# aelmiger/LINE-MOD-Pipeline

Hardware: AMD Instinct MI355X
Metric: detections/sec (higher is better)
Workload: dtype u8

## Files before the change

### line-mod-pipeline_amd/csrc/lm_dev_color.h

```cpp
#pragma once
#include "lm_dev.h"

namespace {

__global__ __launch_bounds__(256) void k_pyrdown(const u8* __restrict__ src0, int sw, int sh, u8* __restrict__ dst0,
                                                  int dw, int dh, size_t slot_stride) {
    const u8* src = slot_ptr(src0, slot_stride);
    u8* dst = slot_ptr(dst0, slot_stride);
    int x = blockIdx.x * 64 + (threadIdx.x & 63);
    int y = blockIdx.y * 4 + (threadIdx.x >> 6);
    if (x >= dw || y >= dh) return;
    const int K[5] = {1, 4, 6, 4, 1};
    int xs[5];
#pragma unroll
    for (int i = 0; i < 5; ++i) xs[i] = refl101(2 * x + i - 2, sw) * 3;
    int s0 = 0, s1 = 0, s2 = 0;
#pragma unroll
    for (int j = 0; j < 5; ++j) {
        const u8* row = src + (size_t)refl101(2 * y + j - 2, sh) * sw * 3;
        int r0 = 0, r1 = 0, r2 = 0;
#pragma unroll
        for (int i = 0; i < 5; ++i) {
            const u8* p = row + xs[i];
            r0 += K[i] * p[0]; r1 += K[i] * p[1]; r2 += K[i] * p[2];
// ... 536 lines not shown
            for (int e = 0; e < 4; ++e) {
                const int j = 4 * q + e, k = 16 * hh + j;
                const int d0 = k - 16 - n, d1 = k + 16 - n;
                const int w0 = (d0 % 3 == 0) ? mx_w(d0 / 3 + 3) : 0, w1 = (d1 % 3 == 0) ? mx_w(d1 / 3 + 3) : 0;
                const int m = (j & 3) + 8 * (j >> 2) + 4 * hh;
                const int yy = m >> 2, cc = m & 3;
                const int wp = cc == cco ? mx_w(yy - yo - 1) : 0, wc = cc == cco ? mx_w(yy - yo + 7) : 0;
                b0 |= (u32)w0 << (8 * e); b1 |= (u32)w1 << (8 * e); vp |= (u32)wp << (8 * e); vc |= (u32)wc << (8 * e);
            }
            T.v[lane][q] = b0; T.v[lane][4 + q] = b1; T.v[lane][8 + q] = vp; T.v[lane][12 + q] = vc;
        }
    }
    return T;
}
__device__ const MxTab g_mx_tab = mx_make_tab();
#define MX_WAVE_BYTES 128
__device__ __forceinline__ void permlane32_swap_lo(u32& a, u32& b) {
    const auto r = __builtin_amdgcn_permlane32_swap(a, b, false, false);
    a = r[0]; b = r[1];
}
__device__ __forceinline__ void d_cblur_mx_st(const u32 slot, const u32 tile, const u8* __restrict__ bgr0, int w, int h, u8* __restrict__ s0, size_t in_stride,
                                              size_t tmp_stride, int gx, int strip_rows) {
    const u8* bgr = slot_ptr_s(bgr0, in_stride, slot);
    u8* S = slot_ptr_s(s0, tmp_stride, slot);
    const int lane = (int)(threadIdx.x & 63u), wave = (int)(threadIdx.x >> 6);
    const int r = lane & 31, hh = lane >> 5;
    const int yy = r >> 2, cc = r & 3;
    const int cx = (int)(tile % (u32)gx), sy = (int)(tile / (u32)gx);
    const int W3 = w * 3;
    const int c0 = (cx * 4 + wave) * MX_WAVE_BYTES;
    if (c0 >= W3) return;
    const int Y0 = sy * strip_rows, Y1 = min(Y0 + strip_rows, h);
    const u32 pitch = (u32)W3;
    i32x4 B0, B1, BP, BC;
    {
        const u32x4* tp = reinterpret_cast<const u32x4*>(g_mx_tab.v[lane]);
        const u32x4 t0 = tp[0], t1 = tp[1], t2 = tp[2], t3 = tp[3];
        B0 = i32x4{(int)t0[0], (int)t0[1], (int)t0[2], (int)t0[3]}; B1 = i32x4{(int)t1[0], (int)t1[1], (int)t1[2], (int)t1[3]};
        BP = i32x4{(int)t2[0], (int)t2[1], (int)t2[2], (int)t2[3]}; BC = i32x4{(int)t3[0], (int)t3[1], (int)t3[2], (int)t3[3]};
    }
    const int cch = c0 + 32 * cc;
    const bool active = cch < W3;
    const bool rep_l = active && cch == 0 && hh == 0;
    const bool rep_r = active && cch + 32 == W3 && hh == 1;
    const bool edge_wave = __any(rep_l || rep_r);
    const u32 off0 = (u32)(!active ? 0 : rep_l ? 0 : cch - 16 + 16 * hh);
    const u32 off1 = (u32)(!active ? 0 : rep_r ? W3 - 16 : cch + 16 + 16 * hh);
    auto load_tile = [&](int yt, u32x4 (&A)[2]) {
        const u32 row = (u32)clampi(yt + yy, 0, h - 1) * pitch;
        u32x4 v0 = ld16(bgr + (row + off0)), v1 = ld16(bgr + (row + off1));
        if (edge_wave) {
            const u32 dl = v0[0], dr = v1[3];
            const u32 l0 = __builtin_amdgcn_perm(dl, dl, 0x02010002u), l1 = __builtin_amdgcn_perm(dl, dl, 0x00020100u), l2 = __builtin_amdgcn_perm(dl, dl, 0x01000201u);
            const u32 r0 = __builtin_amdgcn_perm(dr, dr, 0x01030201u), r1 = __builtin_amdgcn_perm(dr, dr, 0x02010302u), r2 = __builtin_amdgcn_perm(dr, dr, 0x03020103u);
            v0 = rep_l ? u32x4{l0, l1, l2, l0} : v0;
            v1 = rep_r ? u32x4{r0, r1, r2, r0} : v1;
        }
        A[0] = u32x4{v0[0] ^ 0x80808080u, v0[1] ^ 0x80808080u, v0[2] ^ 0x80808080u, v0[3] ^ 0x80808080u};
        A[1] = u32x4{v1[0] ^ 0x80808080u, v1[1] ^ 0x80808080u, v1[2] ^ 0x80808080u, v1[3] ^ 0x80808080u};
    };
    auto horizontal = [&](const u32x4 (&A)[2], i32x4& Hi, i32x4& Lo) {
        i32x16 c = {0, 0, 0, 0, 0, 0, 0, 0, 0, 0, 0, 0, 0, 0, 0, 0};
        c = __builtin_amdgcn_mfma_i32_32x32x32_i8(i32x4{(int)A[0][0], (int)A[0][1], (int)A[0][2], (int)A[0][3]}, B0, c, 0, 0, 0);
        c = __builtin_amdgcn_mfma_i32_32x32x32_i8(i32x4{(int)A[1][0], (int)A[1][1], (int)A[1][2], (int)A[1][3]}, B1, c, 0, 0, 0);
#pragma unroll
        for (int g = 0; g < 4; ++g) {
            const u32 r0 = (u32)c[4 * g], r1 = (u32)c[4 * g + 1], r2 = (u32)c[4 * g + 2], r3 = (u32)c[4 * g + 3];
            const u32 a01 = __builtin_amdgcn_perm(r1, r0, 0x05010400u), a23 = __builtin_amdgcn_perm(r3, r2, 0x05010400u);
            Lo[g] = (int)(__builtin_amdgcn_perm(a23, a01, 0x05040100u) ^ 0x80808080u);
            Hi[g] = (int)__builtin_amdgcn_perm(a23, a01, 0x07060302u);
        }
    };
    u32x4 A[2], An[2];
    i32x4 hiP, loP, hiC, loC;
    load_tile(Y0 - 4, A);
    horizontal(A, hiP, loP);
    const int steps = (Y1 - Y0 + 7) / 8;
    const int KC = 32768 + 128 * 256 + 32768 * 256;
    load_tile(Y0 + 4, A);
    const u32 so = (u32)(cch + 16 * hh);
    for (int m = 0; m < steps; ++m) {
        if (m + 1 < steps) load_tile(Y0 + 8 * (m + 1) + 4, An);
        horizontal(A, hiC, loC);
        i32x16 zh = {0, 0, 0, 0, 0, 0, 0, 0, 0, 0, 0, 0, 0, 0, 0, 0};
        i32x16 zl = {KC, KC, KC, KC, KC, KC, KC, KC, KC, KC, KC, KC, KC, KC, KC, KC};
        zh = __builtin_amdgcn_mfma_i32_32x32x32_i8(hiP, BP, zh, 0, 0, 0);
        zh = __builtin_amdgcn_mfma_i32_32x32x32_i8(hiC, BC, zh, 0, 0, 0);
        zl = __builtin_amdgcn_mfma_i32_32x32x32_i8(loP, BP, zl, 0, 0, 0);
        zl = __builtin_amdgcn_mfma_i32_32x32x32_i8(loC, BC, zl, 0, 0, 0);
        u32 D[4];
#pragma unroll
        for (int g = 0; g < 4; ++g) {
            u32 v[4];
#pragma unroll
            for (int e = 0; e < 4; ++e) v[e] = ((u32)zh[4 * g + e] << 8) + (u32)zl[4 * g + e];
            const u32 a01 = __builtin_amdgcn_perm(v[1], v[0], 0x0c0c0602u), a23 = __builtin_amdgcn_perm(v[3], v[2], 0x0c0c0602u);
            D[g] = __builtin_amdgcn_perm(a23, a01, 0x05040100u);
        }
        permlane32_swap_lo(D[0], D[2]);
        permlane32_swap_lo(D[1], D[3]);
        const int yout = Y0 + 8 * m + yy;
        if (active && yout < Y1) st16(S + ((u32)yout * pitch + so), u32x4{D[0], D[2], D[1], D[3]});
        hiP = hiC; loP = loC;
        A[0] = An[0]; A[1] = An[1];
    }
}

__global__ __launch_bounds__(256, 2) void k_cblur_mx(const u8* __restrict__ bgr0, int w, int h, u8* __restrict__ s0, size_t in_stride,
                                                     size_t tmp_stride, int gx, int gy, int strip_rows, int nslots) {
    u32 slot, tile;
    xcd_slot_tile_b(blockIdx.x, (u32)(gx * gy), (u32)nslots, slot, tile);
    d_cblur_mx_st(slot, tile, bgr0, w, h, s0, in_stride, tmp_stride, gx, strip_rows);
}
__global__ __launch_bounds__(256, 2) void k_blur_mx_pyr(const u8* __restrict__ bgr0, int w, int h, u8* __restrict__ s0, u8* __restrict__ bgr1,
                                                        size_t slot_stride, int gx, int gy, int strip_rows, int g_pyr, int nslots) {
    u32 slot, tile;
    const u32 g_blur = (u32)(gx * gy), G = g_blur + (u32)g_pyr;
    xcd_slot_tile_b(blockIdx.x, G, (u32)nslots, slot, tile);
    const u32 p1 = (tile + 1u) * (u32)g_pyr / G, p0 = tile * (u32)g_pyr / G;
    if (p1 != p0) d_pyrdown16_st<PD_STRIP>(slot, p0, bgr0, w, h, bgr1, w >> 1, h >> 1, slot_stride);
    else d_cblur_mx_st(slot, tile - p0, bgr0, w, h, s0, slot_stride, slot_stride, gx, strip_rows);
}

template <int SB>
__global__ __launch_bounds__(256, 2) void k_blur_pyr(const u8* __restrict__ bgr0, int w, int h, u8* __restrict__ s0, u8* __restrict__ bgr1,
                                                     size_t slot_stride, int g_blur, int g_pyr, int nslots, int interleave) {
    u32 slot, tile;
    xcd_slot_tile_b(blockIdx.x, (u32)(g_blur + g_pyr), (u32)nslots, slot, tile);
    if (!interleave) {
        if (tile < (u32)g_blur) d_cblur_sh_st<SB>(slot, tile, bgr0, w, h, s0, slot_stride, slot_stride);
        else d_pyrdown16_st<PD_STRIP>(slot, tile - (u32)g_blur, bgr0, w, h, bgr1, w >> 1, h >> 1, slot_stride);
        return;
    }
    const u32 G = (u32)(g_blur + g_pyr);
    const u32 p1 = (tile + 1u) * (u32)g_pyr / G, p0 = tile * (u32)g_pyr / G;
    if (p1 != p0) d_pyrdown16_st<PD_STRIP>(slot, p0, bgr0, w, h, bgr1, w >> 1, h >> 1, slot_stride);
    else d_cblur_sh_st<SB>(slot, tile - p0, bgr0, w, h, s0, slot_stride, slot_stride);
}

__device__ __forceinline__ void d_corient(const u32 vblock, const u8* __restrict__ s0, int w, int h, float thr2,
                                                  u8* __restrict__ qn0, float* __restrict__ mag0, size_t tmp_stride,
                                                  size_t mag_stride, int gblocks, int nslots) {
    u32 slot, tile;
    xcd_slot_tile_b(vblock, (u32)gblocks, (u32)nslots, slot, tile);
    const u8* S = slot_ptr_s(s0, tmp_stride, slot);
    u8* qn = slot_ptr_s(qn0, tmp_stride, slot);
    float* mag = mag0 ? slot_ptr_s(mag0, mag_stride, slot) : nullptr;
    const int ng = w >> 4;
    const int gid = (int)(tile * 256u) + (int)threadIdx.x;
    const int y = gid / ng, g = gid - y * ng;
    if (y >= h) return;
    const size_t pitch = (size_t)w * 3;
    u32 R[3][14];
#pragma unroll
    for (int j = 0; j < 3; ++j) {
        const u8* row = S + (size_t)clampi(y - 1 + j, 0, h - 1) * pitch + 48 * g;
        const u32x4 a = ld16(row), b = ld16(row + 16), c = ld16(row + 32);
        R[j][0] = g > 0 ? *reinterpret_cast<const u32*>(row - 4) : 0u;
        R[j][1] = a[0]; R[j][2] = a[1]; R[j][3] = a[2]; R[j][4] = a[3];
        R[j][5] = b[0]; R[j][6] = b[1]; R[j][7] = b[2]; R[j][8] = b[3];
        R[j][9] = c[0]; R[j][10] = c[1]; R[j][11] = c[2]; R[j][12] = c[3];
        R[j][13] = g + 1 < ng ? *reinterpret_cast<const u32*>(row + 48) : 0u;
    }
    u32 vse[14], vso[14], vde[14], vdo[14];
#pragma unroll
    for (int d = 0; d < 14; ++d) {
        const u32 e0 = R[0][d] & 0x00FF00FFu, o0 = (R[0][d] >> 8) & 0x00FF00FFu;
        const u32 e1 = R[1][d] & 0x00FF00FFu, o1 = (R[1][d] >> 8) & 0x00FF00FFu;
        const u32 e2 = R[2][d] & 0x00FF00FFu, o2 = (R[2][d] >> 8) & 0x00FF00FFu;
        vse[d] = e0 + 2u * e1 + e2; vso[d] = o0 + 2u * o1 + o2;
        vde[d] = e2 + 0x01000100u - e0; vdo[d] = o2 + 0x01000100u - o0;
    }
#define LM_WIN(E, O, wb) ((int)((((wb) & 1) ? O[(wb) >> 2] : E[(wb) >> 2]) >> (((wb) & 2) ? 16 : 0)) & 0xFFFF)
    u32 out[4] = {0, 0, 0, 0};
    float fmv[16];
#pragma unroll
    for (int p = 0; p < 16; ++p) {
        const int x = 16 * g + p;
        int bdx = 0, bdy = 0, bm = -1;
#pragma unroll
        for (int c = 0; c < 3; ++c) {
            int sl, sr, dl, dr;
            if (p == 0) {
                sl = g == 0 ? LM_WIN(vse, vso, 1 + 3 * 1 + c) : LM_WIN(vse, vso, 1 + 3 * 0 + c);
                dl = g == 0 ? LM_WIN(vde, vdo, 1 + 3 * 1 + c) : LM_WIN(vde, vdo, 1 + 3 * 0 + c);
            } else {
                sl = LM_WIN(vse, vso, 1 + 3 * p + c);
                dl = LM_WIN(vde, vdo, 1 + 3 * p + c);
            }
            if (p == 15) {
                sr = g == ng - 1 ? LM_WIN(vse, vso, 1 + 3 * 16 + c) : LM_WIN(vse, vso, 1 + 3 * 17 + c);
                dr = g == ng - 1 ? LM_WIN(vde, vdo, 1 + 3 * 16 + c) : LM_WIN(vde, vdo, 1 + 3 * 17 + c);
            } else {
                sr = LM_WIN(vse, vso, 1 + 3 * (p + 2) + c);
                dr = LM_WIN(vde, vdo, 1 + 3 * (p + 2) + c);
            }
            const int dc = LM_WIN(vde, vdo, 1 + 3 * (p + 1) + c);
            const int dx = sr - sl;
            const int dy = dl + 2 * dc + dr - 1024;
            const int m = dx * dx + dy * dy;
            if (m > bm) { bm = m; bdx = dx; bdy = dy; }
        }
        const float scale = (float)(16.0 / 360.0);
        const float ang = fast_atan2_deg((float)bdy, (float)bdx);
        const float qf = rintf(__fadd_rn(__fmul_rn(ang, scale), 0.0f));
        int q = (int)qf;
        q = q < 0 ? 0 : (q > 255 ? 255 : q);
        const bool border = (y == 0) | (y == h - 1) | (x == 0) | (x == w - 1);
        u32 o = border ? 0u : (u32)(q & 7);
        const float fm = (float)bm;
        if (fm > thr2) o |= 0x80u;
        out[p >> 2] |= o << (8 * (p & 3));
        fmv[p] = fm;
    }
#undef LM_WIN
    st16(qn + (size_t)y * w + 16 * g, u32x4{out[0], out[1], out[2], out[3]});
    if (mag) {
        float* mo = mag + (size_t)y * w + 16 * g;
#pragma unroll
        for (int p = 0; p < 16; ++p) mo[p] = fmv[p];
    }
}
__global__ __launch_bounds__(256) void k_corient(const u8* __restrict__ s0, int w, int h, float thr2,
                                                  u8* __restrict__ qn0, float* __restrict__ mag0, size_t tmp_stride,
                                                  size_t mag_stride, int gblocks, int nslots) {
    d_corient(blockIdx.x, s0, w, h, thr2, qn0, mag0, tmp_stride, mag_stride, gblocks, nslots);
}

#define CVT_ROWS 4
__device__ __forceinline__ void d_cvote(const u32 vblock, const u8* __restrict__ qn0, int w, int h, u8* __restrict__ quant0,
                                                size_t tmp_stride, size_t out_stride, int gblocks, int nslots) {
    u32 slot, tile;
    xcd_slot_tile_b(vblock, (u32)gblocks, (u32)nslots, slot, tile);
    const u8* qn = slot_ptr_s(qn0, tmp_stride, slot);
    u8* quant = slot_ptr_s(quant0, out_stride, slot);
    const int ng = w >> 4;
    const int gid = (int)(tile * 256u) + (int)threadIdx.x;
    const int band = gid / ng, g = gid - band * ng;
    const int y0 = band * CVT_ROWS;
    if (y0 >= h) return;
    u32 hs[3][16];
    u32 flags[3][4];
#pragma unroll
    for (int i = 0; i < CVT_ROWS + 2; ++i) {
        const int yy = clampi(y0 - 1 + i, 0, h - 1);
        const u8* row = qn + (size_t)yy * w + 16 * g;
        const u32x4 c = ld16(row);
        const u32 lft = g > 0 ? *reinterpret_cast<const u32*>(row - 4) : 0u;
        const u32 rgt = g + 1 < ng ? *reinterpret_cast<const u32*>(row + 16) : 0u;
        u32 oh[18];
        oh[0] = 1u << (((lft >> 24) & 7u) << 2);
#pragma unroll
        for (int k = 0; k < 16; ++k) oh[1 + k] = 1u << (((c[k >> 2] >> (8 * (k & 3))) & 7u) << 2);
        oh[17] = 1u << ((rgt & 7u) << 2);
#pragma unroll
        for (int k = 0; k < 16; ++k) hs[i % 3][k] = oh[k] + oh[k + 1] + oh[k + 2];
#pragma unroll
        for (int k = 0; k < 4; ++k) flags[i % 3][k] = c[k];
        if (i >= 2) {
            const int y = y0 + i - 2;
            if (y < h) {
                u32 o[4] = {0, 0, 0, 0};
                const bool yin = y >= 1 && y <= h - 2;
#pragma unroll
                for (int k = 0; k < 16; ++k) {
                    const u32 cnt = hs[0][k] + hs[1][k] + hs[2][k];
                    const u32 m = (cnt + 0x33333333u) & 0x88888888u;
                    const u32 fl = (flags[(i - 1) % 3][k >> 2] >> (8 * (k & 3))) & 0x80u;
                    const int x = 16 * g + k;
                    const bool ok = yin && x >= 1 && x <= w - 2 && fl && m;
                    const u32 res = ok ? (1u << ((u32)(__ffs((int)m) - 1) >> 2)) : 0u;
                    o[k >> 2] |= res << (8 * (k & 3));
                }
                st16(quant + (size_t)y * w + 16 * g, u32x4{o[0], o[1], o[2], o[3]});
            }
        }
    }
}
__global__ __launch_bounds__(256) void k_cvote(const u8* __restrict__ qn0, int w, int h, u8* __restrict__ quant0,
                                                size_t tmp_stride, size_t out_stride, int gblocks, int nslots) {
    d_cvote(blockIdx.x, qn0, w, h, quant0, tmp_stride, out_stride, gblocks, nslots);
}

typedef short s16x2 __attribute__((ext_vector_type(2)));
__device__ __forceinline__ u32 pk_sub_i16(u32 a, u32 b) {
    return __builtin_bit_cast(u32, (s16x2)(__builtin_bit_cast(s16x2, a) - __builtin_bit_cast(s16x2, b)));
}
__device__ __forceinline__ u32 pk_add_i16(u32 a, u32 b) {
    return __builtin_bit_cast(u32, (s16x2)(__builtin_bit_cast(s16x2, a) + __builtin_bit_cast(s16x2, b)));
}
__device__ __forceinline__ u32 pk_max_i16(u32 a, u32 b) {
    return __builtin_bit_cast(u32, __builtin_elementwise_max(__builtin_bit_cast(s16x2, a), __builtin_bit_cast(s16x2, b)));
}
__device__ __forceinline__ int dot2_i16(u32 p, u32 k) {
    int r;
    asm("v_dot2_i32_i16 %0, %1, %2, 0" : "=v"(r) : "v"(p), "s"(k));
    return r;
}
__device__ __forceinline__ int dot2_self(u32 p) {
    int r;
    asm("v_dot2_i32_i16 %0, %1, %1, 0" : "=v"(r) : "v"(p));
    return r;
}
struct CgRow { u32 E[14], O[14]; };
struct CgRaw { u32x4 a, b, c; u32 l, r; };
__device__ __forceinline__ void cg_request(CgRaw& q, const u8* S, int y, int h, u32 pitch, u32 so, u32 lo, u32 ro) {
    const u32 row = (u32)clampi(y, 0, h - 1) * pitch;
    q.a = ld16(S + (row + so)); q.b = ld16(S + (row + so + 16u)); q.c = ld16(S + (row + so + 32u));
    q.l = *reinterpret_cast<const u32*>(S + (row + lo)); q.r = *reinterpret_cast<const u32*>(S + (row + ro));
}
__device__ __forceinline__ void cg_unpack(CgRow& u, const CgRaw& q) {
    const u32 R[14] = {q.l, q.a[0], q.a[1], q.a[2], q.a[3], q.b[0], q.b[1], q.b[2], q.b[3], q.c[0], q.c[1], q.c[2], q.c[3], q.r};
#pragma unroll
    for (int d = 0; d < 14; ++d) {
        u.E[d] = __builtin_amdgcn_perm(R[d], R[d], 0x0c020c00u);
        u.O[d] = __builtin_amdgcn_perm(R[d], R[d], 0x0c030c01u);
    }
}
__device__ __forceinline__ void cg_labels(const CgRow& A, const CgRow& B, const CgRow& N, u32 lmask, bool first, bool last,
                                          int ithr, u32 (&oh)[16], u32& fw) {
    u32 vse[14], vso[14], vde[14], vdo[14];
#pragma unroll
    for (int d = 0; d < 14; ++d) {
        vse[d] = A.E[d] + N.E[d] + 2u * B.E[d]; vso[d] = A.O[d] + N.O[d] + 2u * B.O[d];
        vde[d] = pk_sub_i16(N.E[d], A.E[d]); vdo[d] = pk_sub_i16(N.O[d], A.O[d]);
    }
    u32 P[56];
    int M[56];
    u32 He[13], Ho[13];
#pragma unroll
    for (int d = 0; d <= 12; ++d) {
        He[d] = pk_add_i16(vde[d], __builtin_amdgcn_alignbit(vdo[d + 1], vdo[d], 16));
        Ho[d] = pk_add_i16(vdo[d], vde[d + 1]);
    }
#pragma unroll
    for (int d = 1; d <= 12; ++d) {
        const u32 dxe = pk_sub_i16(__builtin_amdgcn_alignbit(vso[d + 1], vso[d], 16), vso[d - 1]);
        const u32 dxo = pk_sub_i16(vse[d + 1], __builtin_amdgcn_alignbit(vse[d], vse[d - 1], 16));
        const u32 dye = pk_add_i16(Ho[d - 1], He[d]);
        const u32 dyo = pk_add_i16(__builtin_amdgcn_alignbit(He[d], He[d - 1], 16), Ho[d]);
        P[4 * d + 0] = __builtin_amdgcn_perm(dye, dxe, 0x05040100u); P[4 * d + 1] = __builtin_amdgcn_perm(dyo, dxo, 0x05040100u);
        P[4 * d + 2] = __builtin_amdgcn_perm(dye, dxe, 0x07060302u); P[4 * d + 3] = __builtin_amdgcn_perm(dyo, dxo, 0x07060302u);
#pragma unroll
        for (int k = 0; k < 4; ++k) M[4 * d + k] = dot2_self(P[4 * d + k]);
    }
    fw = 0;
#pragma unroll
    for (int p = 0; p < 16; ++p) {
        const int wb = 4 + 3 * p;
        const int m0 = M[wb], m1 = M[wb + 1], m2 = M[wb + 2];
        const int bm = max(max(m0, m1), m2);
        const u32 p0 = P[wb], p1 = P[wb + 1], p2 = P[wb + 2];
        u32 W = m1 >= m2 ? p1 : p2;
        W = m0 == bm ? p0 : W;
        const u32 Aa = pk_max_i16(W, pk_sub_i16(0u, W));
        u32 sg = 0;
        sg = __builtin_amdgcn_alignbit(sg, (u32)dot2_i16(Aa, 255u | (((u32)-1282 & 0xFFFFu) << 16)), 31);
        sg = __builtin_amdgcn_alignbit(sg, (u32)dot2_i16(Aa, 925u | (((u32)-1384 & 0xFFFFu) << 16)), 31);
        sg = __builtin_amdgcn_alignbit(sg, (u32)dot2_i16(Aa, 1384u | (((u32)-925 & 0xFFFFu) << 16)), 31);
        sg = __builtin_amdgcn_alignbit(sg, (u32)dot2_i16(Aa, 1282u | (((u32)-255 & 0xFFFFu) << 16)), 31);
        int q = __builtin_popcount(sg);
        q = ((W ^ (W >> 16)) & 0x8000u) ? -q : q;
        u32 sh = ((u32)q << 2) & lmask;
        if (p == 0) sh = first ? 0u : sh;
        if (p == 15) sh = last ? 0u : sh;
        oh[p] = 1u << sh;
        fw = __builtin_amdgcn_alignbit(fw, (u32)(ithr - bm), 31);
    }
}

#define CG_STRIP 16
template <int STRIP>
__device__ __forceinline__ void d_cgrad(const u32 vblock, const u8* __restrict__ s0, int w, int h, int ithr, u8* __restrict__ quant0,
                                        size_t tmp_stride, size_t out_stride, int gblocks, int nslots) {
    u32 slot, tile;
    xcd_slot_tile_b(vblock, (u32)gblocks, (u32)nslots, slot, tile);
    const u8* S = slot_ptr_s(s0, tmp_stride, slot);
    u8* quant = slot_ptr_s(quant0, out_stride, slot);
    const int ns = w >> 4, total = ns * ((h + STRIP - 1) / STRIP);
    const int lane = (int)(threadIdx.x & 63u);
    const int f0 = ((int)tile * 4 + (int)(threadIdx.x >> 6)) * 62 - 1;
    if (f0 + 1 >= total) return;
    const bool writer = lane >= 1 && lane <= 62 && f0 + lane < total;
    const int f = clampi(f0 + lane, 0, total - 1);
    const int strip = f / ns, g = f - strip * ns;
    const int y0 = strip * STRIP;
    const u32 pitch = (u32)w * 3u;
    const u32 so = 48u * (u32)g;
    const u32 lo = g > 0 ? so - 4u : so, ro = g + 1 < ns ? so + 48u : so + 44u;
    const bool first = g == 0, last = g == ns - 1;
    CgRow R[3];
    {
        CgRaw q0, q1;
        cg_request(q0, S, y0 - 2, h, pitch, so, lo, ro);
        cg_request(q1, S, y0 - 1, h, pitch, so, lo, ro);
        cg_unpack(R[0], q0); cg_unpack(R[1], q1);
    }
    CgRaw nx;
    cg_request(nx, S, y0, h, pitch, so, lo, ro);
    u32 H[3][16], F[3] = {0, 0, 0};
#pragma unroll
    for (int p = 0; p < 16; ++p) { H[0][p] = 0; H[1][p] = 0; H[2][p] = 0; }
    const u32 emask = 0xFFFFu & ~((first ? 0x8000u : 0u) | (last ? 1u : 0u));
#define CG_STEP(K)                                                                                          \
    {                                                                                                       \
        const int r = y0 - 1 + t + (K);                                         \
        cg_unpack(R[((K) + 2) % 3], nx);                                                                    \
        cg_request(nx, S, r + 2, h, pitch, so, lo, ro);                         \
        u32 oh[16];                                                                                         \
        cg_labels(R[(K) % 3], R[((K) + 1) % 3], R[((K) + 2) % 3], (r <= 0 || r >= h - 1) ? 0u : 28u, first, last, ithr, oh, F[((K) + 2) % 3]); \
        const u32 ohl = (u32)__builtin_amdgcn_update_dpp(0, (int)oh[15], 0x138, 0xf, 0xf, true);    \
        const u32 ohr = (u32)__builtin_amdgcn_update_dpp(0, (int)oh[0], 0x130, 0xf, 0xf, true);      \
        _Pragma("unroll") for (int p = 0; p < 16; ++p)                                                      \
            H[((K) + 2) % 3][p] = (p == 0 ? ohl : oh[p - 1]) + oh[p] + (p == 15 ? ohr : oh[p + 1]);         \
        const int y = r - 1;                                    \
        if (t + (K) >= 2 && y < h) {                                                                        \
            const u32 keep = (y >= 1 && y <= h - 2) ? (F[((K) + 1) % 3] & emask) : 0u;                      \
            u32 res[16];                                                                                    \
            _Pragma("unroll") for (int p = 0; p < 16; ++p) {                                                \
                const u32 cnt = H[0][p] + H[1][p] + H[2][p];                                                \
                const u32 m = (cnt + 0x33333333u) & 0x88888888u;    \
                   \
                const u32 one = 1u << (((u32)(__ffs((int)m) - 1) >> 2) & 31u);                              \
                res[p] = one & (u32)__builtin_amdgcn_sbfe((int)keep, 15 - p, 1);                            \
            }                                                                                               \
            u32 o[4];                                                                                       \
            _Pragma("unroll") for (int k = 0; k < 4; ++k)                                                   \
                o[k] = __builtin_amdgcn_perm(__builtin_amdgcn_perm(res[4 * k + 3], res[4 * k + 2], 0x0c0c0400u), \
                                             __builtin_amdgcn_perm(res[4 * k + 1], res[4 * k], 0x0c0c0400u), 0x05040100u); \
            if (writer) st16(quant + ((u32)y * (u32)w + 16u * (u32)g), u32x4{o[0], o[1], o[2], o[3]});      \
        }                                                                                                   \
    }
#pragma unroll 1
    for (int t = 0; t < STRIP + 2; t += 3) {
        CG_STEP(0)
        if (t + 1 >= STRIP + 2) break;
        CG_STEP(1)
        if (t + 2 >= STRIP + 2) break;
        CG_STEP(2)
    }
#undef CG_STEP
}
template <int STRIP>
__global__ __launch_bounds__(256, 2) void k_cgrad(const u8* __restrict__ s0, int w, int h, int ithr, u8* __restrict__ quant0,
                                                  size_t tmp_stride, size_t out_stride, int gblocks, int nslots) {
    d_cgrad<STRIP>(blockIdx.x, s0, w, h, ithr, quant0, tmp_stride, out_stride, gblocks, nslots);
}

template <int S0, int S1>
__global__ __launch_bounds__(256, 2) void k_cgrad_levels(const u8* __restrict__ s0, int w0, int h0, u8* __restrict__ q0, int g0,
                                                         const u8* __restrict__ s1, int w1, int h1, u8* __restrict__ q1, int g1,
                                                         int ithr, size_t slot_stride, int nslots) {
    const u32 e0 = (u32)g0 * (u32)nslots;
    if (blockIdx.x < e0) d_cgrad<S0>(blockIdx.x, s0, w0, h0, ithr, q0, slot_stride, slot_stride, g0, nslots);
    else d_cgrad<S1>(blockIdx.x - e0, s1, w1, h1, ithr, q1, slot_stride, slot_stride, g1, nslots);
}


}
```

Measured before the change: 198,300.

## Compute color-gradient Sobel sums with int8 MFMA using constant weight tables

Replaces the packed-int16 VALU Sobel computation in the color gradient stage with int8 32x32x32 MFMA instructions. Pixel bytes are bias-flipped to signed and multiplied against a per-lane constant weight table, which is built at compile time and held in device memory, to produce the dx/dy sums. Loads change to four 16-byte reads per row, and edge replication is handled in the unpack step. The aim is to move the arithmetic-heavy gradient work onto the matrix cores. In exchange it adds table loads, more registers and MFMA latency, and the sign flip and table indexing must stay exact.

```diff
diff --git a/line-mod-pipeline_amd/csrc/lm_dev_color.h b/line-mod-pipeline_amd/csrc/lm_dev_color.h
--- a/line-mod-pipeline_amd/csrc/lm_dev_color.h
+++ b/line-mod-pipeline_amd/csrc/lm_dev_color.h
@@ -862,70 +862,92 @@
     asm("v_dot2_i32_i16 %0, %1, %1, 0" : "=v"(r) : "v"(p));
     return r;
 }
-struct CgRow { u32 E[14], O[14]; };
-struct CgRaw { u32x4 a, b, c; u32 l, r; };
+struct CgTab { u32 v[64][8][4]; };
+static constexpr int cg_wx(int d) { return d == 3 ? 1 : d == -3 ? -1 : 0; }
+static constexpr int cg_wy(int d) { return (d == 3 || d == -3) ? 1 : d == 0 ? 2 : 0; }
+static constexpr CgTab cg_make_tab() {
+    CgTab T{};
+    for (int lane = 0; lane < 64; ++lane) {
+        const int m = lane & 31, hh = lane >> 5;
+        const bool own = ((m >> 2) & 1) == hh;
+        const int i = (m & 3) + 4 * (m >> 3);
+        for (int c = 0; c < 2; ++c)
+            for (int q = 0; q < 4; ++q) {
+                u32 x1 = 0, x2 = 0, yp = 0, yn = 0;
+                for (int e = 0; e < 4; ++e) {
+                    const int d = 16 * c - 8 + 4 * q + e - i;
+                    const int wx = own ? cg_wx(d) : 0, wy = own ? cg_wy(d) : 0;
+                    x1 |= (u32)(wx & 0xFF) << (8 * e); x2 |= (u32)((2 * wx) & 0xFF) << (8 * e);
+                    yp |= (u32)(wy & 0xFF) << (8 * e); yn |= (u32)((-wy) & 0xFF) << (8 * e);
+                }
+                T.v[lane][c][q] = x1; T.v[lane][2 + c][q] = x2; T.v[lane][4 + c][q] = yp; T.v[lane][6 + c][q] = yn;
+            }
+    }
+    return T;
+}
+__device__ const CgTab g_cg_tab = cg_make_tab();
+struct CgRow { i32x4 p[4]; };
+struct CgRaw { u32x4 p[4]; };
 __device__ __forceinline__ void cg_request(CgRaw& q, const u8* S, int y, int h, u32 pitch, u32 so, u32 lo, u32 ro) {
     const u32 row = (u32)clampi(y, 0, h - 1) * pitch;
-    q.a = ld16(S + (row + so)); q.b = ld16(S + (row + so + 16u)); q.c = ld16(S + (row + so + 32u));
-    q.l = *reinterpret_cast<const u32*>(S + (row + lo)); q.r = *reinterpret_cast<const u32*>(S + (row + ro));
-}
-__device__ __forceinline__ void cg_unpack(CgRow& u, const CgRaw& q) {
-    const u32 R[14] = {q.l, q.a[0], q.a[1], q.a[2], q.a[3], q.b[0], q.b[1], q.b[2], q.b[3], q.c[0], q.c[1], q.c[2], q.c[3], q.r};
-#pragma unroll
-    for (int d = 0; d < 14; ++d) {
-        u.E[d] = __builtin_amdgcn_perm(R[d], R[d], 0x0c020c00u);
-        u.O[d] = __builtin_amdgcn_perm(R[d], R[d], 0x0c030c01u);
-    }
-}
-__device__ __forceinline__ void cg_labels(const CgRow& A, const CgRow& B, const CgRow& N, u32 lmask, bool first, bool last,
+    q.p[0] = ld16a4(S + (row + lo)); q.p[1] = ld16a4(S + (row + so + 8u)); q.p[2] = ld16a4(S + (row + so + 24u)); q.p[3] = ld16a4(S + (row + ro));
+}
+__device__ __forceinline__ void cg_unpack(CgRow& u, const CgRaw& q, bool edge_wave, bool first, bool last) {
+#pragma unroll
+    for (int k = 0; k < 4; ++k)
+        u.p[k] = i32x4{(int)(q.p[k][0] ^ 0x80808080u), (int)(q.p[k][1] ^ 0x80808080u), (int)(q.p[k][2] ^ 0x80808080u), (int)(q.p[k][3] ^ 0x80808080u)};
+    if (edge_wave) {
+        u.p[0][2] = first ? u.p[0][0] : u.p[0][2]; u.p[0][3] = first ? u.p[0][1] : u.p[0][3];
+        u.p[3][0] = last ? u.p[3][2] : u.p[3][0]; u.p[3][1] = last ? u.p[3][3] : u.p[3][1];
+    }
+}
+__device__ __forceinline__ void cg_labels(const CgRow& A, const CgRow& B, const CgRow& N, const i32x4 (&T)[8], u32 lmask, bool first, bool last,
                                           int ithr, u32 (&oh)[16], u32& fw) {
-    u32 vse[14], vso[14], vde[14], vdo[14];
-#pragma unroll
-    for (int d = 0; d < 14; ++d) {
-        vse[d] = A.E[d] + N.E[d] + 2u * B.E[d]; vso[d] = A.O[d] + N.O[d] + 2u * B.O[d];
-        vde[d] = pk_sub_i16(N.E[d], A.E[d]); vdo[d] = pk_sub_i16(N.O[d], A.O[d]);
-    }
-    u32 P[56];
-    int M[56];
-    u32 He[13], Ho[13];
-#pragma unroll
-    for (int d = 0; d <= 12; ++d) {
-        He[d] = pk_add_i16(vde[d], __builtin_amdgcn_alignbit(vdo[d + 1], vdo[d], 16));
-        Ho[d] = pk_add_i16(vdo[d], vde[d + 1]);
-    }
-#pragma unroll
-    for (int d = 1; d <= 12; ++d) {
-        const u32 dxe = pk_sub_i16(__builtin_amdgcn_alignbit(vso[d + 1], vso[d], 16), vso[d - 1]);
-        const u32 dxo = pk_sub_i16(vse[d + 1], __builtin_amdgcn_alignbit(vse[d], vse[d - 1], 16));
-        const u32 dye = pk_add_i16(Ho[d - 1], He[d]);
-        const u32 dyo = pk_add_i16(__builtin_amdgcn_alignbit(He[d], He[d - 1], 16), Ho[d]);
-        P[4 * d + 0] = __builtin_amdgcn_perm(dye, dxe, 0x05040100u); P[4 * d + 1] = __builtin_amdgcn_perm(dyo, dxo, 0x05040100u);
-        P[4 * d + 2] = __builtin_amdgcn_perm(dye, dxe, 0x07060302u); P[4 * d + 3] = __builtin_amdgcn_perm(dyo, dxo, 0x07060302u);
-#pragma unroll
-        for (int k = 0; k < 4; ++k) M[4 * d + k] = dot2_self(P[4 * d + k]);
-    }
+    u32 P[48];
+    int M[48];
     fw = 0;
 #pragma unroll
-    for (int p = 0; p < 16; ++p) {
-        const int wb = 4 + 3 * p;
-        const int m0 = M[wb], m1 = M[wb + 1], m2 = M[wb + 2];
-        const int bm = max(max(m0, m1), m2);
-        const u32 p0 = P[wb], p1 = P[wb + 1], p2 = P[wb + 2];
-        u32 W = m1 >= m2 ? p1 : p2;
-        W = m0 == bm ? p0 : W;
-        const u32 Aa = pk_max_i16(W, pk_sub_i16(0u, W));
-        u32 sg = 0;
-        sg = __builtin_amdgcn_alignbit(sg, (u32)dot2_i16(Aa, 255u | (((u32)-1282 & 0xFFFFu) << 16)), 31);
-        sg = __builtin_amdgcn_alignbit(sg, (u32)dot2_i16(Aa, 925u | (((u32)-1384 & 0xFFFFu) << 16)), 31);
-        sg = __builtin_amdgcn_alignbit(sg, (u32)dot2_i16(Aa, 1384u | (((u32)-925 & 0xFFFFu) << 16)), 31);
-        sg = __builtin_amdgcn_alignbit(sg, (u32)dot2_i16(Aa, 1282u | (((u32)-255 & 0xFFFFu) << 16)), 31);
-        int q = __builtin_popcount(sg);
-        q = ((W ^ (W >> 16)) & 0x8000u) ? -q : q;
-        u32 sh = ((u32)q << 2) & lmask;
-        if (p == 0) sh = first ? 0u : sh;
-        if (p == 15) sh = last ? 0u : sh;
-        oh[p] = 1u << sh;
-        fw = __builtin_amdgcn_alignbit(fw, (u32)(ithr - bm), 31);
+    for (int j = 0; j < 3; ++j) {
+        i32x16 ax = {0, 0, 0, 0, 0, 0, 0, 0, 0, 0, 0, 0, 0, 0, 0, 0}, ay = {0, 0, 0, 0, 0, 0, 0, 0, 0, 0, 0, 0, 0, 0, 0, 0};
+#pragma unroll
+        for (int c = 0; c < 2; ++c) {
+            ax = __builtin_amdgcn_mfma_i32_32x32x32_i8(T[c], A.p[j + c], ax, 0, 0, 0);
+            ay = __builtin_amdgcn_mfma_i32_32x32x32_i8(T[6 + c], A.p[j + c], ay, 0, 0, 0);
+        }
+#pragma unroll
+        for (int c = 0; c < 2; ++c) {
+            ax = __builtin_amdgcn_mfma_i32_32x32x32_i8(T[c], N.p[j + c], ax, 0, 0, 0);
+            ay = __builtin_amdgcn_mfma_i32_32x32x32_i8(T[4 + c], N.p[j + c], ay, 0, 0, 0);
+        }
+#pragma unroll
+        for (int c = 0; c < 2; ++c) ax = __builtin_amdgcn_mfma_i32_32x32x32_i8(T[2 + c], B.p[j + c], ax, 0, 0, 0);
+#pragma unroll
+        for (int i = 0; i < 16; ++i) {
+            P[16 * j + i] = __builtin_amdgcn_perm((u32)ay[i], (u32)ax[i], 0x05040100u);
+            M[16 * j + i] = dot2_self(P[16 * j + i]);
+        }
+#pragma unroll
+        for (int p = 5 * j; p < (j == 2 ? 16 : 5 * j + 5); ++p) {
+            const int wb = 3 * p;
+            const int m0 = M[wb], m1 = M[wb + 1], m2 = M[wb + 2];
+            const int bm = max(max(m0, m1), m2);
+            const u32 p0 = P[wb], p1 = P[wb + 1], p2 = P[wb + 2];
+            u32 W = m1 >= m2 ? p1 : p2;
+            W = m0 == bm ? p0 : W;
+            const u32 Aa = pk_max_i16(W, pk_sub_i16(0u, W));
+            u32 sg = 0;
+            sg = __builtin_amdgcn_alignbit(sg, (u32)dot2_i16(Aa, 255u | (((u32)-1282 & 0xFFFFu) << 16)), 31);
+            sg = __builtin_amdgcn_alignbit(sg, (u32)dot2_i16(Aa, 925u | (((u32)-1384 & 0xFFFFu) << 16)), 31);
+            sg = __builtin_amdgcn_alignbit(sg, (u32)dot2_i16(Aa, 1384u | (((u32)-925 & 0xFFFFu) << 16)), 31);
+            sg = __builtin_amdgcn_alignbit(sg, (u32)dot2_i16(Aa, 1282u | (((u32)-255 & 0xFFFFu) << 16)), 31);
+            int q = __builtin_popcount(sg);
+            q = ((W ^ (W >> 16)) & 0x8000u) ? -q : q;
+            u32 sh = ((u32)q << 2) & lmask;
+            if (p == 0) sh = first ? 0u : sh;
+            if (p == 15) sh = last ? 0u : sh;
+            oh[p] = 1u << sh;
+            fw = __builtin_amdgcn_alignbit(fw, (u32)(ithr - bm), 31);
+        }
     }
 }
 
@@ -947,14 +969,21 @@
     const int y0 = strip * STRIP;
     const u32 pitch = (u32)w * 3u;
     const u32 so = 48u * (u32)g;
-    const u32 lo = g > 0 ? so - 4u : so, ro = g + 1 < ns ? so + 48u : so + 44u;
     const bool first = g == 0, last = g == ns - 1;
+    const bool edge_wave = __any(first || last);
+    const u32 lo = first ? so : so - 8u, ro = last ? so + 32u : so + 40u;
+    i32x4 T[8];
+    {
+        const u32x4* tp = reinterpret_cast<const u32x4*>(g_cg_tab.v[lane]);
+#pragma unroll
+        for (int k = 0; k < 8; ++k) { const u32x4 t = tp[k]; T[k] = i32x4{(int)t[0], (int)t[1], (int)t[2], (int)t[3]}; }
+    }
     CgRow R[3];
     {
         CgRaw q0, q1;
         cg_request(q0, S, y0 - 2, h, pitch, so, lo, ro);
         cg_request(q1, S, y0 - 1, h, pitch, so, lo, ro);
-        cg_unpack(R[0], q0); cg_unpack(R[1], q1);
+        cg_unpack(R[0], q0, edge_wave, first, last); cg_unpack(R[1], q1, edge_wave, first, last);
     }
     CgRaw nx;
     cg_request(nx, S, y0, h, pitch, so, lo, ro);
@@ -965,10 +994,10 @@
 #define CG_STEP(K)                                                                                          \
     {                                                                                                       \
         const int r = y0 - 1 + t + (K);                                         \
-        cg_unpack(R[((K) + 2) % 3], nx);                                                                    \
+        cg_unpack(R[((K) + 2) % 3], nx, edge_wave, first, last);                                                                  \
         cg_request(nx, S, r + 2, h, pitch, so, lo, ro);                         \
         u32 oh[16];                                                                                         \
-        cg_labels(R[(K) % 3], R[((K) + 1) % 3], R[((K) + 2) % 3], (r <= 0 || r >= h - 1) ? 0u : 28u, first, last, ithr, oh, F[((K) + 2) % 3]); \
+        cg_labels(R[(K) % 3], R[((K) + 1) % 3], R[((K) + 2) % 3], T, (r <= 0 || r >= h - 1) ? 0u : 28u, first, last, ithr, oh, F[((K) + 2) % 3]); \
         const u32 ohl = (u32)__builtin_amdgcn_update_dpp(0, (int)oh[15], 0x138, 0xf, 0xf, true);    \
         const u32 ohr = (u32)__builtin_amdgcn_update_dpp(0, (int)oh[0], 0x130, 0xf, 0xf, true);      \
         _Pragma("unroll") for (int p = 0; p < 16; ++p)                                                      \
```

New measurement: 199,100 (median of 6 runs). No clear change (+0.4%).
